# ACMEAtronOmatic/DSen2

Hardware: AMD Instinct MI355X
Metric: 32x32x6 patches/sec (DSen2_20, d=6, batch 512) (higher is better)
Workload: dtype f32; 1 GPU; DSen2_20 d=6 F=128 fp32, 512 synthetic 32x32 patches (4+6 bands) per GPU per step, he_uniform random-init weights; batch_per_gpu=512, parallelism=patch-sharded dp1, backend=rccl, output_gather=False

## Files before the change

### dsen2_amd/_lib.py

```python
import ctypes
import os
import sys

_HERE = os.path.dirname(os.path.abspath(__file__))
LIB_PATH = os.environ.get('DSEN2_HIP_LIB') or os.path.join(_HERE, 'libdsen2_hip.so')

OK = 0
ERR_INVALID, ERR_HIP, ERR_NO_WEIGHTS, ERR_WORKSPACE, ERR_NO_DEVICE, ERR_NOMEM, ERR_INTERNAL = -1, -2, -3, -4, -5, -6, -7
DTYPE_U16, DTYPE_F32 = 0, 1
DTYPE_F64 = 2
MASK_BLANK_MAP = 3

c_float_p = ctypes.POINTER(ctypes.c_float)
c_int_p = ctypes.POINTER(ctypes.c_int)
c_void_p = ctypes.c_void_p
c_int = ctypes.c_int
c_size_t = ctypes.c_size_t
c_double = ctypes.c_double


class CorpusTile(ctypes.Structure):
    _fields_ = [('dev_lr10', c_void_p), ('dev_lr20', c_void_p), ('dev_lr60', c_void_p), ('dev_gt', c_void_p),
                ('grid_h', c_int), ('grid_w', c_int), ('gt_dtype', c_int)]


SIGNATURES = {
    'dsen2_version': (ctypes.c_char_p, []),
    'dsen2_last_error': (ctypes.c_char_p, []),
    'dsen2_device_count': (c_int, []),
    'dsen2_model_create': (c_int, [ctypes.POINTER(c_void_p), c_int, c_int, c_int, c_int, c_int, c_int]),
    'dsen2_model_destroy': (None, [c_void_p]),
    'dsen2_model_num_params': (c_size_t, [c_void_p]),
    'dsen2_model_load_weights': (c_int, [c_void_p, c_float_p, c_size_t]),
    'dsen2_model_workspace_bytes': (c_int, [c_void_p, c_int, c_int, c_int, ctypes.POINTER(c_size_t)]),
    'dsen2_model_forward': (c_int, [c_void_p, c_void_p, c_void_p, c_void_p, c_void_p, c_int, c_int, c_int,
                                    c_void_p, c_size_t, c_void_p]),
    'dsen2_model_body_launches': (c_int, [c_void_p, c_int, c_int, c_int]),
    'dsen2_dihedral_nchw': (c_int, [c_void_p, c_void_p, c_int, c_int, c_int, c_int, c_int, c_void_p, c_int, c_void_p]),
    'dsen2_dihedral_accumulate': (c_int, [c_void_p, c_void_p, c_int, c_int, c_int, c_int, c_int, c_int, c_void_p]),
    'dsen2_model_ensemble_workspace_bytes': (c_int, [c_void_p, c_int, c_int, c_int, c_int, ctypes.POINTER(c_size_t)]),
    'dsen2_model_forward_ensemble': (c_int, [c_void_p, c_void_p, c_void_p, c_void_p, c_void_p, c_int, c_int, c_int, c_int,
                                             c_void_p, c_size_t, c_void_p]),
    'dsen2_model_forward_timed': (c_int, [c_void_p, c_void_p, c_void_p, c_void_p, c_void_p, c_int, c_int, c_int,
                                          c_void_p, c_size_t, c_void_p, c_int, c_float_p]),
    'dsen2_model_forward_profile': (c_int, [c_void_p, c_void_p, c_void_p, c_void_p, c_void_p, c_int, c_int, c_int,
                                            c_void_p, c_size_t, c_void_p, c_int, c_int, c_float_p]),
    'dsen2_conv3x3_nhwc': (c_int, [c_void_p, c_float_p, c_float_p, c_void_p, c_void_p, c_int, c_int, c_int, c_int,
                                   c_int, c_int, ctypes.c_float, c_void_p]),
    'dsen2_conv3x3_nhwc_ref': (c_int, [c_void_p, c_float_p, c_float_p, c_void_p, c_void_p, c_int, c_int, c_int, c_int,
                                       c_int, c_int, ctypes.c_float, c_void_p]),
    'dsen2_split_f32': (c_int, [c_void_p, c_void_p, c_void_p, c_int, c_int, c_int, c_int, c_void_p]),
    'dsen2_join_f32': (c_int, [c_void_p, c_void_p, c_void_p, c_int, c_int, c_int, c_int, c_void_p]),
# ... 142 lines not shown
```

### dsen2_amd/asm_contract.py

```python
import os
import re
import subprocess
import tempfile

HERE = os.path.dirname(os.path.abspath(__file__))
CSRC = os.path.join(HERE, 'csrc')
DMA_SOURCES = ['conv3x3_body32.hip', 'conv3x3_body16w.hip']


class AsmContractError(RuntimeError):
    pass


def _code_lines(text):
    return [ln.strip() for ln in text.splitlines() if ln.strip() and not ln.strip().startswith((';', '.', '//'))]


def _kernels(text):
    out, name, body = {}, None, []
    for ln in text.splitlines():
        m = re.match(r'^(_Z\w+):', ln)
        if m:
            name, body = m.group(1), []
            continue
# ... 97 lines not shown
            n_dma = [sum(1 for ln in c if ln.startswith('buffer_load_dword') and ln.endswith('lds')) for c in copies]
            need(min(n_dma) == 0 and max(n_dma) > 0, 'kernel %s: DMAs in both copies of the item loop' % name, n_dma)
            quiet, loud = (copies[0], copies[1]) if n_dma[0] == 0 else (copies[1], copies[0])
            need(not any(re.search(r'\bm0\b', ln) for ln in quiet), 'kernel %s: M0 use in the compute-only copy' % name)
            run = None
            for ln in loud:
                if re.match(r's_mov_b32 (s\d+|vcc_lo|vcc_hi), m0$', ln):
                    need(run is None, 'kernel %s: M0 saved twice in one DMA statement' % name)
                    run = 0
                elif ln.startswith('buffer_load_dword') and ln.endswith('lds'):
                    need(run is not None, 'kernel %s: DMA outside a statement that saves M0' % name)
                    run += 1
                elif run and not re.match(r'(s_mov_b32 m0, |s_nop 0$)', ln):
                    need(run in (2, 4), 'kernel %s: a DMA statement of %d instructions' % (name, run))
                    run = None
    if src == 'conv3x3_body16w.hip':
        expect = {0: (0, 32), 1: (64, 64), 3: (64, 64)}
        expect3 = {0: (0, 64), 1: (64, 96), 3: (64, 64)}

        def count(pattern, want, msg, product=lambda m: True):
            found = []
            for name, body in kernels.items():
                m = re.search(pattern, name)
                if not m or not product(m):
                    continue
                found.append(body)
                loads = sum(1 for ln in body if ln.startswith('buffer_load_dwordx4') and not ln.endswith('lds'))
                stores = sum(1 for ln in body if ln.startswith('buffer_store_dwordx4'))
                need((loads, stores) == want(m), msg(m) % (loads, stores, want(m)))
            return found
# ... 49 lines not shown
        need(not any(ln.startswith('global_store') for ln in body), 'kernel %s stores outside its buffer descriptors' % name)
        mf = [i for i, ln in enumerate(body) if ln.startswith('v_mfma')]
        need(mf, 'kernel %s has no MFMA' % name)
        x3 = 'ELb1EEE' in name
        floor = 24 if x3 else 16
        loop = body[mf[0]:]
        scat = [i for i, ln in enumerate(loop) if ln.startswith('ds_write_b16')]
        need(scat, 'kernel %s: no halo scatter after the first MFMA' % name)
        waits = [ln for ln in loop[:scat[-1]] if ln.startswith('s_waitcnt') and 'vmcnt' in ln]
        low = [ln for ln in waits if int(re.search(r'vmcnt\((\d+)\)', ln).group(1)) < floor]
        need(not low, 'kernel %s: a wait inside the tile loop drains the deferred stores (divergent branch in the loop body?)' % name, low[:4])
    return True


TRAFFIC_KERNELS = {
    'dsen2_20_fp32': ('conv3x3_body32.hip', r'conv3x3_body32_kernelILi128ELi128ELi0ELi0ELi0ELi4ELb1E'),
    'vdsen2_20_bf16': ('conv3x3_body16w.hip', r'conv3x3_body16w_chain_kernelILi128ELi256ELi0E'),
    'dsen2_20_bf16x3': ('conv3x3_body16w.hip', r'conv3x3_body16w_x3_chain_kernelILi64ELi128E'),
    'vdsen2_20_fp32': ('conv3x3_body32.hip', r'conv3x3_body32_kernelILi256ELi256ELi0ELi0ELi0ELi4ELb1E'),
    'dsen2_20_bf16': ('conv3x3_body16w.hip', r'conv3x3_body16w_chain_kernelILi64ELi128ELi0E'),
    'vdsen2_20_bf16x3': ('conv3x3_body16w.hip', r'conv3x3_body16w_x3_chain_kernelILi128ELi256E'),
}
ISA_JSON = os.path.join(HERE, 'kernel_isa.json')


def isa_hashes(text):
    import hashlib
    out = {}
    for name, body in _kernels(text).items():
        out[name] = hashlib.sha256('\n'.join(normalised(body)).encode()).hexdigest()
    return out
# ... 32 lines not shown
```

### dsen2_amd/csrc/capi.hip

```cpp

#include <chrono>
#include <cstdarg>
#include <cstdio>
#include <cstring>
#include <exception>
#include <new>
#include <vector>

#include "capi_internal.h"

using namespace dsen2;

namespace {

thread_local char g_err[512] = "";

#ifdef DSEN2_DIAG
Tuning g_diag_tuning;
unsigned long long* g_diag_stamps = nullptr;
#endif
Tuning default_tuning() {
#ifdef DSEN2_DIAG
  return g_diag_tuning;
#else
// ... 4 lines not shown
constexpr int kWarmLaunches = 24;

}

namespace dsen2 {
int fail(int code, const char* fmt, ...) {
  va_list ap;
  va_start(ap, fmt);
  vsnprintf(g_err, sizeof(g_err), fmt, ap);
  va_end(ap);
  return code;
}
}

static bool may_chain(const dsen2_model* m) {
  return m->chain_stride != 0 && m->tune.chain && m->tune.grid_cap == 0 && (m->precision == 1 || m->tune.ablate == 0);
}

static int first_layer(const dsen2_model* m, const float* x10, const float* x20, const float* x60, int n, int h, int w,
                       const ForwardWs& B, bool x0_packed, hipStream_t stream) {
  const Layer& L = m->layers[0];
  const ConvPlan& pl = L.plan;
  const float* P = m->dev_params;
  const bool x3 = m->precision == 2 && m->num_layers > 0;
  ConvParams pf = make_params(B.x0, L.weights(P), L.bias(P), nullptr, B.a, n, h, w, 0, 0.f);
  if (pl.epilogue == kEpiReluSplit) {
    pf.out = reinterpret_cast<float*>(B.s0);
    pf.out2 = B.s1;
  }
  const FirstInputs fi{x60, m->c10, m->c20, m->c60};
  ConvParams pd = pf;
// ... 81 lines not shown

int forward_launches(const dsen2_model* m, const float* x10, const float* x20, const float* x60, float* out, int n, int h, int w,
                     const ForwardWs& B, size_t keep_step, bool x0_packed, hipStream_t stream, const hipEvent_t* ev) {
  const float* P = m->dev_params;
  const int d = m->num_layers;
  if (ev) HIP_TRY(hipEventRecord(ev[0], stream));
  if (int rc = first_layer(m, x10, x20, x60, n, h, w, B, x0_packed, stream)) return rc;
  if (ev) HIP_TRY(hipEventRecord(ev[1], stream));
  if (m->precision != 0 && d > 0) {
    if (keep_step > 0) {
      HIP_TRY((m->precision == 2 ? launch_join3_f32 : launch_join_f32)(B.s0, B.s1, B.x0f, n, h, w, m->feat, stream));
      HIP_TRY(hipMemcpyAsync(B.xkeep, B.s0, operand16_bytes(m, n, h, w), hipMemcpyDeviceToDevice, stream));
    }
    if (int rc = body16(m, B.s0, B.s1, B.t16, B.a, n, h, w, stream, keep_step, B.xkeep)) return rc;
  } else {
    for (int l = 1; l <= d; ++l) {
      const Layer& LA = m->layers[2 * l - 1];
      const Layer& LB = m->layers[2 * l];
      const float* x_in = B.a + (size_t)(l - 1) * keep_step;
      float* t = B.t + (size_t)(l - 1) * keep_step;
      HIP_TRY(launch(LA.plan, make_params(x_in, LA.weights(P), LA.bias(P), nullptr, t, n, h, w, 0, 0.f), LA.plan.epilogue, m->tune, stream));
      HIP_TRY(launch(LB.plan, make_params(t, LB.weights(P), LB.bias(P), x_in, B.a + (size_t)l * keep_step, n, h, w, 0, 0.1f),
                     LB.plan.epilogue, m->tune, stream));
    }
  }
  if (ev) HIP_TRY(hipEventRecord(ev[2], stream));
  {
    const Layer& L = m->layers.back();
    const float* skip = m->c60 > 0 ? x60 : x20;
    const float* x_d = B.a + (m->precision == 0 ? (size_t)d * keep_step : 0);
    ConvParams po = make_params(x_d, L.weights(P), L.bias(P), skip, out, n, h, w, m->cout, 0.f);
// ... 355 lines not shown
}

int dsen2_model_forward(dsen2_model* m, const float* x10, const float* x20, const float* x60, float* out, int n, int h, int w,
                        void* workspace, size_t workspace_bytes, void* stream) {
  return guarded([&] { return forward(m, x10, x20, x60, out, n, h, w, workspace, workspace_bytes, stream, nullptr); });
}

int dsen2_model_body_launches(const dsen2_model* m, int n, int h, int w) {
  return guarded([&]() -> int {
    if (!m) return fail(DSEN2_ERR_INVALID, "NULL model");
    if (int rc = check_shape(m, n, h, w)) return rc;
    if (int rc = check_device(m)) return rc;
    int dev = 0, cus = 0;
    if (hipGetDevice(&dev) != hipSuccess || hipDeviceGetAttribute(&cus, hipDeviceAttributeMultiprocessorCount, dev) != hipSuccess)
      return fail(DSEN2_ERR_NO_DEVICE, "no HIP device");
    return may_chain(m) && body16w_chain_patches_per_wg(n, h, w, m->feat, cus) > 0 ? 1 : 2 * m->num_layers;
  });
}

int dsen2_model_forward_timed(dsen2_model* m, const float* x10, const float* x20, const float* x60, float* out, int n, int h, int w,
                              void* workspace, size_t workspace_bytes, void* stream, int iters, float* body_ms_per_launch) {
  return guarded([&]() -> int {
    if (!body_ms_per_launch) return fail(DSEN2_ERR_INVALID, "NULL result");
    if (!m || m->num_layers <= 0) return fail(DSEN2_ERR_INVALID, "model has no residual blocks");
    float ms[5];
    int rc = forward_profile(m, x10, x20, x60, out, n, h, w, workspace, workspace_bytes, stream, 0, iters, ms);
    if (rc == DSEN2_OK) *body_ms_per_launch = ms[2] / (2.0f * m->num_layers);
    return rc;
  });
}

int dsen2_model_forward_profile(dsen2_model* m, const float* x10, const float* x20, const float* x60, float* out, int n, int h,
// ... 208 lines not shown
```

### dsen2_amd/csrc/conv3x3_body32.hip

```cpp
#include <type_traits>

#include "conv3x3_dma.h"

namespace dsen2 {

namespace {

using dma::KC; using dma::NT; using dma::THREADS; using dma::QS; using dma::IN_BYTES; using dma::IN_BLOCKS;
using dma::WCH; using dma::NWBUF; using dma::LDS_BYTES; using dma::wait_vmcnt;
constexpr int KSTEPS = 4;
constexpr int PB = 2, MB = 2;
static_assert((8 * kHalo) % 16 == 0, "rows R and R+8 of a pixel block sit on the same banks");

}

template <int CIN, int COUT, int EPI, int ABL, int PRE, int STG, bool DEFER>
__global__ __launch_bounds__(THREADS, 2) void conv3x3_body32_kernel(const ConvParams p, const int n_items) {
  constexpr int NCC = CIN / KC;
  constexpr int NS = COUT / NT;
  static_assert(NCC % 2 == 0, "input double buffer parity");
  constexpr bool ASYM = STG >= 2;
  using Stage = dma::Stage<CIN, NS, false, ASYM ? dma::Role::Issuer : dma::Role::All>;
  constexpr int N_W = (ABL & 4) ? 0 : Stage::N_W;

// ... 246 lines not shown
    } else {
      if constexpr ((STG - 2) / KSTEPS == 1) __builtin_amdgcn_s_setprio(1);
      run(std::integral_constant<int, 0>{}, std::false_type{});
    }
  } else if constexpr (STG == 1) {
    if (wave < 4)
      run(std::integral_constant<int, 0>{}, std::true_type{});
    else
      run(std::integral_constant<int, KSTEPS / 2>{}, std::true_type{});
  } else {
    run(std::integral_constant<int, 0>{}, std::true_type{});
  }
  wait_vmcnt<0>();
}

template <int CIN, int COUT, int EPI, int ABL = 0, int PRE = 0, int STG = 0, bool DEFER = false>
static hipError_t launch_body32_one(const ConvParams& p, hipStream_t stream) {
  const long long items = (long long)p.n * p.tiles_x * p.tiles_y * (COUT / NT);
  return launch_persistent<conv3x3_body32_kernel<CIN, COUT, EPI, ABL, PRE, STG, DEFER>>(LDS_BYTES, THREADS, items, 1, 0, stream, p);
}

constexpr int kAsym = 2 + KSTEPS / 2;

template <int F>
static hipError_t launch_body32_feat(const ConvParams& p, int epilogue, Body32Form form, hipStream_t stream) {
  const bool relu = epilogue == kEpiRelu;
#ifdef DSEN2_DIAG
  if (form == Body32Form::Plain || form == Body32Form::StaggerA) {
    if (!relu) return launch_body32_one<F, F, kEpiResidual, 0, 2, 0>(p, stream);
    return form == Body32Form::Plain ? launch_body32_one<F, F, kEpiRelu, 0, 0, 0>(p, stream) : launch_body32_one<F, F, kEpiRelu, 0, 0, 1>(p, stream);
  }
  if (form == Body32Form::DeferStaggerA && !relu) return launch_body32_one<F, F, kEpiResidual, 0, 0, 0, true>(p, stream);
  if (form == Body32Form::DeferStagger || form == Body32Form::DeferStaggerA)
    return relu ? launch_body32_one<F, F, kEpiRelu, 0, 0, 1, true>(p, stream) : launch_body32_one<F, F, kEpiResidual, 0, 0, 1, true>(p, stream);
#define DSEN2_ASYM(FORM, STG)                                                                                      \
  if (form == Body32Form::FORM)                                                                                    \
    return relu ? launch_body32_one<F, F, kEpiRelu, 0, 0, STG, true>(p, stream) : launch_body32_one<F, F, kEpiResidual, 0, 0, STG, true>(p, stream);
// ... 35 lines not shown
```

### dsen2_amd/csrc/conv3x3_dma.h

```cpp
#pragma once
#include "conv3x3_items.h"

namespace dsen2 {
namespace dma {

constexpr int KC = 32;
constexpr int NT = 128;
constexpr int THREADS = 512;
constexpr int QS = 336;
constexpr int IN_BYTES = 8 * QS * 16;
constexpr int IN_BLOCKS = 6;
constexpr int WCH = KC * NT;
constexpr int NWBUF = 4;
constexpr size_t LDS_BYTES = (size_t)2 * IN_BYTES + (size_t)NWBUF * WCH * 4 + 256 * 4;
static_assert(QS >= kHaloPix && QS % 16 == 0 && 64 * (IN_BLOCKS - 1) + 16 == QS, "input chunk geometry");
static_assert(LDS_BYTES <= 160 * 1024, "LDS budget");

template <int N>
__device__ __forceinline__ void wait_vmcnt() {
  static_assert(N >= 0 && N <= 63, "vmcnt is a 6-bit field");
  asm volatile("s_waitcnt vmcnt(%0)" ::"n"(N) : "memory");
}

__device__ __forceinline__ unsigned lds_address(const float* p) {
  return (unsigned)(size_t)(__attribute__((address_space(3))) const float*)p;
}

enum class Role { All, Issuer };

template <int CINW, int NS, bool LAZY_VOFF = false, Role ROLE = Role::All>
struct Stage {
// ... 23 lines not shown
    in_rsrc = __builtin_amdgcn_make_buffer_rsrc(const_cast<float*>(p.in), 0, 0, 0x00020000);
    w_rsrc = __builtin_amdgcn_make_buffer_rsrc(const_cast<float*>(p.wpk), 0, (unsigned)(NS * NCHUNK * WCH * 4), 0x00020000);
    w_voff = lane * 16;
    wl_item = lid; wl_chunk = 0; st_slot = 0;
    st_y0 = st_x0 = 0;
  }

  __device__ __forceinline__ unsigned voff_of(int b, int ty0, int tx0) const {
    const int hp = 64 * b + lane;
    const int hy = hp / kHalo, hx = hp - hy * kHalo;
    const int gy = ty0 - 1 + hy, gx = tx0 - 1 + hx;
    const bool inb = hp < kHaloPix && (unsigned)gy < (unsigned)h && (unsigned)gx < (unsigned)w;
    return inb ? (unsigned)(((gy * w + gx) * CINW + wave * 4) * 4) : 0x80000000u;
  }

  __device__ __forceinline__ void set_stage_item(int item) {
    const Tile t = tile_at<NS>(item, tiles_per_img, tiles_x);
    in_rsrc = __builtin_amdgcn_make_buffer_rsrc(const_cast<float*>(in) + (size_t)t.img * img_pix * CINW, 0,
                                                (unsigned)(img_pix * CINW * 4), 0x00020000);
    if constexpr (LAZY_VOFF) {
      st_y0 = t.ty0;
      st_x0 = t.tx0;
    } else {
#pragma unroll
      for (int b = 0; b < IN_BLOCKS; ++b) in_voff[b] = voff_of(b, t.ty0, t.tx0);
    }
  }

  __device__ __forceinline__ void issue_in(int buf, int b, int cc) {
    const unsigned m0v = lds_in + buf * IN_BYTES + (wave * QS + 64 * b) * 16;
    const unsigned so = cc * (KC * 4);
    const unsigned voff = LAZY_VOFF ? voff_of(b, st_y0, st_x0) : in_voff[LAZY_VOFF ? 0 : b];
    if constexpr (ROLE == Role::Issuer) {
// ... 13 lines not shown
                     : "=&s"(saved_m0) : "s"(m0v), "s"(m1v), "v"(voff), "s"(in_rsrc), "s"(so), "s"(so1) : "memory");
      }
      return;
    }
    unsigned saved_m0;
    if (b < IN_BLOCKS - 1) {
      asm volatile("s_mov_b32 %0, m0\n\ts_mov_b32 m0, %1\n\ts_nop 0\n\tbuffer_load_dwordx4 %2, %3, %4 offen lds\n\ts_mov_b32 m0, %0"
                   : "=&s"(saved_m0) : "s"(m0v), "v"(voff), "s"(in_rsrc), "s"(so) : "memory");
    } else if (lane < 16) {
      asm volatile("s_mov_b32 %0, m0\n\ts_mov_b32 m0, %1\n\ts_nop 0\n\tbuffer_load_dwordx4 %2, %3, %4 offen lds\n\ts_mov_b32 m0, %0"
                   : "=&s"(saved_m0) : "s"(m0v), "v"(voff), "s"(in_rsrc), "s"(so) : "memory");
    }
  }

  __device__ __forceinline__ void issue_w() {
    const unsigned so = (unsigned)(((wl_item % NS) * NCHUNK + wl_chunk) * (WCH * 4) + wave * 1024);
    const unsigned l0 = lds_w + st_slot * (WCH * 4) + wave * 1024;
    unsigned saved_m0;
    if constexpr (ROLE == Role::Issuer)
      asm volatile(
          "s_mov_b32 %0, m0\n\t"
          "s_mov_b32 m0, %1\n\ts_nop 0\n\tbuffer_load_dwordx4 %5, %6, %7 offen lds\n\t"
          "s_mov_b32 m0, %2\n\ts_nop 0\n\tbuffer_load_dwordx4 %5, %6, %8 offen lds\n\t"
          "s_mov_b32 m0, %3\n\ts_nop 0\n\tbuffer_load_dwordx4 %5, %6, %9 offen lds\n\t"
          "s_mov_b32 m0, %4\n\ts_nop 0\n\tbuffer_load_dwordx4 %5, %6, %10 offen lds\n\t"
          "s_mov_b32 m0, %0"
          : "=&s"(saved_m0)
          : "s"(l0), "s"(l0 + 4096u), "s"(l0 + 8192u), "s"(l0 + 12288u), "v"(w_voff), "s"(w_rsrc), "s"(so), "s"(so + 4096u),
            "s"(so + 8192u), "s"(so + 12288u)
          : "memory");
    else
    asm volatile(
        "s_mov_b32 %0, m0\n\t"
        "s_mov_b32 m0, %1\n\ts_nop 0\n\tbuffer_load_dwordx4 %3, %4, %5 offen lds\n\t"
        "s_mov_b32 m0, %2\n\ts_nop 0\n\tbuffer_load_dwordx4 %3, %4, %6 offen lds\n\t"
        "s_mov_b32 m0, %0"
        : "=&s"(saved_m0) : "s"(l0), "s"(l0 + 8192u), "v"(w_voff), "s"(w_rsrc), "s"(so), "s"(so + 8192u)
        : "memory");
    if (++wl_chunk == NCHUNK) {
      wl_chunk = 0;
      wl_item = wl_item + G < n_items ? wl_item + G : lid;
    }
    st_slot = st_slot == NWBUF - 1 ? 0 : st_slot + 1;
  }
};

}
}
```

### dsen2_amd/csrc/conv_plan.h

```cpp
#pragma once
#include <vector>

#include "dsen2_internal.h"

namespace dsen2 {

enum class ConvRole { First, BodyA, BodyB, Output, DgradBody, DgradOutput };
enum class ConvKernel {
  Tile,
  Body32,
  Body16,
  Body16x3,
  Out
};

constexpr size_t kAlignFloats = 64;
inline size_t align_up(size_t v) { return (v + kAlignFloats - 1) / kAlignFloats * kAlignFloats; }

struct ConvPlan {
  ConvRole role;
  ConvKernel kernel;
  int epilogue;
  int cin, cout;
  int cin_pad, cout_pad;
// ... 15 lines not shown

struct Layer {
  ConvPlan plan;
  size_t off, flat_off;
  const float* weights(const float* params) const { return params + off; }
  const float* bias(const float* params) const { return params + off + plan.bias_off; }
  const float* first16(const float* params) const { return params + off + plan.first16_off; }
};
struct NetworkPlan {
  std::vector<Layer> layers;
  size_t n_params = 0;
  size_t dev_param_floats = 0;
  size_t chain_stride = 0;
};
bool plan_network(int c10, int c20, int c60, int num_layers, int feat, int precision, const Tuning& tune, NetworkPlan* net);

}
```

### dsen2_amd/csrc/conv_plan.hip

```cpp
#include <cstring>
#include <vector>

#include "conv_plan.h"

namespace dsen2 {

namespace {

constexpr int kBody16Chunk = 32;

bool sentinel2(const BandGroups* b) { return b && b->c10 == 4 && b->c20 == 6 && (b->c60 == 0 || b->c60 == 2); }

void pack_tile_weights(const float* k, const ConvPlan& pl, float* dst) {
  const int ncc = pl.cin_pad / pl.kc, nslab = pl.cout_pad / pl.nt, ng = pl.kc / 4;
  size_t i = 0;
  for (int slab = 0; slab < nslab; ++slab)
    for (int cc = 0; cc < ncc; ++cc)
      for (int tap = 0; tap < 9; ++tap)
        for (int gg = 0; gg < ng; ++gg)
          for (int o = 0; o < pl.nt; ++o)
            for (int j = 0; j < 4; ++j, ++i) {
              const int c = cc * pl.kc + 4 * gg + j, oc = slab * pl.nt + o;
              dst[i] = (c < pl.cin && oc < pl.cout) ? k[((size_t)tap * pl.cin + c) * pl.cout + oc] : 0.f;
            }
// ... 75 lines not shown
      pl.kernel = precision == 1   ? ConvKernel::Body16
                  : precision == 2 ? ConvKernel::Body16x3
                  : tune.body == BodyKernel::Body32 ? ConvKernel::Body32 : ConvKernel::Tile;
      break;
  }
  const size_t taps = tap_floats(pl);
  pl.weight_floats = pl.kernel == ConvKernel::Body16     ? taps / 2
                     : pl.kernel == ConvKernel::Body16x3 ? 3 * taps / 2
                                                         : taps + (pl.out_mfma ? out_mfma_weight_floats(cin) : 0);
  pl.bias_off = align_up(pl.weight_floats);
  pl.floats = pl.first16_off = pl.bias_off + align_up((size_t)pl.cout_pad);
  if (pl.first16_planes) pl.floats += align_up((first16_weight_u16(cout, pl.first16_planes == 2) + 1) / 2);
  return true;
}

void pack(const ConvPlan& pl, const float* k, const float* bias, float* dst) {
  memset(dst, 0, sizeof(float) * (bias ? pl.floats : pl.weight_floats));
  switch (pl.kernel) {
    case ConvKernel::Tile:
    case ConvKernel::Body32: pack_tile_weights(k, pl, dst); break;
    case ConvKernel::Body16: pack_conv_weights_bf16_host(k, pl.cin, pl.cout, reinterpret_cast<uint16_t*>(dst)); break;
    case ConvKernel::Body16x3: pack_conv_weights_bf16x3_host(k, pl.cin, pl.cout, reinterpret_cast<uint16_t*>(dst)); break;
    case ConvKernel::Out:
      pack_out_valu_weights_host(k, pl.cin, pl.cout, dst);
      if (pl.out_mfma) pack_out_mfma_weights_host(k, pl.cin, pl.cout, dst + tap_floats(pl));
      break;
  }
  if (!bias) return;
  memcpy(dst + pl.bias_off, bias, sizeof(float) * pl.cout);
  if (pl.first16_planes)
// ... 26 lines not shown
  *net = NetworkPlan{};
  auto add = [&](ConvRole role, int ci, int co, int prec) {
    Layer L;
    if (!plan_conv(role, ci, co, prec, tune, &bands, &L.plan)) return false;
    L.flat_off = net->n_params;
    net->n_params += (size_t)9 * ci * co + co;
    L.off = net->dev_param_floats;
    net->dev_param_floats += L.plan.floats;
    net->layers.push_back(L);
    return true;
  };
  if (!add(ConvRole::First, c10 + c20 + c60, feat, num_layers > 0 ? precision : 0)) return false;
  for (int i = 0; i < num_layers; ++i)
    if (!add(ConvRole::BodyA, feat, feat, precision) || !add(ConvRole::BodyB, feat, feat, precision)) return false;
  if (!add(ConvRole::Output, feat, c60 > 0 ? c60 : c20, 0)) return false;
  if (num_layers > 0 && precision != 0) net->chain_stride = net->layers[1].plan.floats * sizeof(float);
  return true;
}

}
```

### dsen2_amd/csrc/dsen2_internal.h

```cpp
#pragma once
#include <hip/hip_runtime.h>
#include <stddef.h>
#include <stdint.h>

#include <mutex>

namespace dsen2 {


constexpr int kTile = 16;
constexpr int kHalo = kTile + 2;
constexpr int kHaloPix = kHalo * kHalo;

enum Epilogue : int {
  kEpiRelu = 0, kEpiResidual = 1, kEpiSkipNCHW = 2,
  kEpiResidualF32 = 3,
  kEpiReluSplit = 4
};

struct ConvParams {
  const float* in;
  const float* wpk;
  const float* bias;
  const float* aux;
// ... 62 lines not shown
hipError_t launch_conv3x3_body16w(const ConvParams& p, int feat, int epilogue, bool x3, int ablate, hipStream_t stream, int grid_cap = 0);
hipError_t launch_split3_f32(const float* in_nhwc, void* hx, void* lo, int n, int h, int w, int c, hipStream_t stream);
struct ChainArgs {
  void* hi;
  void* lo;
  void* t;
  float* out_f32;
  unsigned layer_stride;
  int n_layers;
  int patches_per_wg;
  int seamless;
};
hipError_t launch_conv3x3_body16w_chain(const ConvParams& p, const ChainArgs& c, int feat, hipStream_t stream, int ablate = 0,
                                        bool x3 = false);
int body16w_chain_patches_per_wg(int n, int h, int w, int feat, int cus);
hipError_t launch_split_f32(const float* in_nhwc, void* hi, void* lo, int n, int h, int w, int c, hipStream_t stream);
hipError_t launch_join_f32(const void* hi, const void* lo, float* out_nhwc, int n, int h, int w, int c, hipStream_t stream);
inline uint16_t f32_to_bf16_rne(float f) {
  uint32_t u = __builtin_bit_cast(uint32_t, f);
  if ((u & 0x7fffffffu) > 0x7f800000u) return (uint16_t)((u >> 16) | 0x40);
  u += 0x7fffu + ((u >> 16) & 1u);
  return (uint16_t)(u >> 16);
}

hipError_t launch_pack_inputs(const float* x10, const float* x20, const float* x60, int c10, int c20, int c60,
                              float* out_nhwc16, int n, int h, int w, hipStream_t stream);
hipError_t launch_upsample(const float* in, float* out, int planes, int h, int w, int oh, int ow, float post_div,
                           hipStream_t stream, bool general = false);
hipError_t launch_tile_gather(const float* img, int H, int W, int C, int border, const int* origins, int count,
                              int P, float divisor, float* patches, hipStream_t stream);
// ... 65 lines not shown
```

### include/dsen2_hip.h

```cpp
#ifndef DSEN2_HIP_H
#define DSEN2_HIP_H

#include <stddef.h>

#ifdef __cplusplus
extern "C" {
#endif

#define DSEN2_OK 0
#define DSEN2_ERR_INVALID (-1)
#define DSEN2_ERR_HIP (-2)
#define DSEN2_ERR_NO_WEIGHTS (-3)
#define DSEN2_ERR_WORKSPACE (-4)
#define DSEN2_ERR_NO_DEVICE (-5)
#define DSEN2_ERR_NOMEM (-6)
#define DSEN2_ERR_INTERNAL (-7)

typedef struct dsen2_model dsen2_model;

const char *dsen2_version(void);
const char *dsen2_last_error(void);
int dsen2_device_count(void);

int dsen2_model_create(dsen2_model **out, int c10, int c20, int c60, int num_layers, int feature_size,
                       int precision);
void dsen2_model_destroy(dsen2_model *m);

size_t dsen2_model_num_params(const dsen2_model *m);

int dsen2_model_load_weights(dsen2_model *m, const float *host_flat, size_t count);

int dsen2_model_workspace_bytes(const dsen2_model *m, int n, int h, int w, size_t *bytes);

int dsen2_model_forward(dsen2_model *m, const float *dev_x10, const float *dev_x20, const float *dev_x60,
                        float *dev_out, int n, int h, int w, void *dev_workspace, size_t workspace_bytes,
                        void *stream);

int dsen2_model_body_launches(const dsen2_model *m, int n, int h, int w);

int dsen2_model_forward_timed(dsen2_model *m, const float *x10, const float *x20, const float *x60, float *out,
                              int n, int h, int w, void *workspace, size_t workspace_bytes, void *stream, int iters,
                              float *body_ms_per_launch);

int dsen2_model_forward_profile(dsen2_model *m, const float *x10, const float *x20, const float *x60, float *out,
                                int n, int h, int w, void *workspace, size_t workspace_bytes, void *stream, int warm,
                                int iters, float *ms5);

int dsen2_dihedral_nchw(const float *dev_in, float *dev_out, int n, int c, int h, int w, int op, const int *dev_ops_or_null,
                        int inverse, void *stream);
int dsen2_dihedral_accumulate(const float *dev_in, float *dev_acc, int n, int c, int h, int w, int op, int count_or_0,
                              void *stream);
int dsen2_model_ensemble_workspace_bytes(const dsen2_model *m, int n, int h, int w, int mask, size_t *bytes);
int dsen2_model_forward_ensemble(dsen2_model *m, const float *dev_x10, const float *dev_x20, const float *dev_x60,
// ... 165 lines not shown
```

Baseline: 40390 patches/s.

## Fuse fp32 residual-block body layers into one persistent chained kernel

Adds a persistent fp32 chain kernel that runs all 2*d body convolutions in a single launch. Each workgroup owns a fixed set of patches and walks layer by layer, ping-ponging activations between two buffers. It prefetches the next layer's weights and bias via LDS DMA while overlapping the previous item's epilogue (bias, ReLU or residual add) with the current MFMA loop. The aim is to remove per-layer launch overhead and tail imbalance for small 32x32 patches. The cost is that each workgroup must stay on its patches, so occupancy is limited to n/ppw workgroups, and the kernel is only enabled when the layout heuristic accepts it.

```diff
diff --git a/dsen2_amd/_lib.py b/dsen2_amd/_lib.py
--- a/dsen2_amd/_lib.py
+++ b/dsen2_amd/_lib.py
@@ -36,6 +36,7 @@
     'dsen2_model_forward': (c_int, [c_void_p, c_void_p, c_void_p, c_void_p, c_void_p, c_int, c_int, c_int,
                                     c_void_p, c_size_t, c_void_p]),
     'dsen2_model_body_launches': (c_int, [c_void_p, c_int, c_int, c_int]),
+    'dsen2_chain_patches_per_workgroup': (c_int, [c_int, c_int, c_int, c_int, c_int, c_int]),
     'dsen2_dihedral_nchw': (c_int, [c_void_p, c_void_p, c_int, c_int, c_int, c_int, c_int, c_void_p, c_int, c_void_p]),
     'dsen2_dihedral_accumulate': (c_int, [c_void_p, c_void_p, c_int, c_int, c_int, c_int, c_int, c_int, c_void_p]),
     'dsen2_model_ensemble_workspace_bytes': (c_int, [c_void_p, c_int, c_int, c_int, c_int, ctypes.POINTER(c_size_t)]),
diff --git a/dsen2_amd/asm_contract.py b/dsen2_amd/asm_contract.py
--- a/dsen2_amd/asm_contract.py
+++ b/dsen2_amd/asm_contract.py
@@ -135,6 +135,33 @@
                 elif run and not re.match(r'(s_mov_b32 m0, |s_nop 0$)', ln):
                     need(run in (2, 4), 'kernel %s: a DMA statement of %d instructions' % (name, run))
                     run = None
+        chains = {k: v for k, v in kernels.items() if re.search(r'conv3x3_body32_chain_kernelILi(128|256)E', k)}
+        need(len(chains) == 2, 'expected the 2 instantiations of the fp32 chain kernel, found %d' % len(chains))
+        for name, body in chains.items():
+            need(not any('scratch_' in ln or ln.startswith(('v_writelane_b32', 'v_readlane_b32')) for ln in body),
+                 'kernel %s spills registers' % name)
+            mf = [i for i, ln in enumerate(body) if ln.startswith('v_mfma')]
+            need(len(mf) == 2 * ITEM_MFMAS, 'kernel %s: %d MFMAs, expected two copies of the item loop' % (name, len(mf)))
+            copies = [body[mf[0]:mf[ITEM_MFMAS - 1]], body[mf[ITEM_MFMAS]:mf[-1]]]
+            n_dma = [sum(1 for ln in c if ln.startswith('buffer_load_dword') and ln.endswith('lds')) for c in copies]
+            need(min(n_dma) == 0 and max(n_dma) > 0, 'kernel %s: DMAs in both copies of the item loop' % name, n_dma)
+            quiet, loud = (copies[0], copies[1]) if n_dma[0] == 0 else (copies[1], copies[0])
+            need(not any(re.search(r'\bm0\b', ln) for ln in quiet), 'kernel %s: M0 use in the compute-only copy' % name)
+            need(any(ln.startswith('s_waitcnt') and re.search(r'vmcnt\(0\)', ln) for ln in quiet),
+                 'kernel %s: the compute-only copy never retires its own stores' % name)
+            run = None
+            for ln in loud:
+                if re.match(r's_mov_b32 (s\d+|vcc_lo|vcc_hi), m0$', ln):
+                    need(run is None, 'kernel %s: M0 saved twice in one DMA statement' % name)
+                    run = 0
+                elif ln.startswith('buffer_load_dword') and ln.endswith('lds'):
+                    need(run is not None, 'kernel %s: DMA outside a statement that saves M0' % name)
+                    run += 1
+                elif run and not re.match(r'(s_mov_b32 m0, |s_nop 0$)', ln):
+                    need(run in (1, 2, 4), 'kernel %s: a DMA statement of %d instructions' % (name, run))
+                    run = None
+            waits = [int(m.group(1)) for ln in loud for m in [re.search(r'^s_waitcnt vmcnt\((\d+)\)$', ln)] if m]
+            need(waits.count(6) >= 12 and waits.count(4) >= 6, 'kernel %s: the issuers\' counted step waits are gone' % name, waits[:20])
     if src == 'conv3x3_body16w.hip':
         expect = {0: (0, 32), 1: (64, 64), 3: (64, 64)}
         expect3 = {0: (0, 64), 1: (64, 96), 3: (64, 64)}
@@ -214,7 +241,7 @@
 
 
 TRAFFIC_KERNELS = {
-    'dsen2_20_fp32': ('conv3x3_body32.hip', r'conv3x3_body32_kernelILi128ELi128ELi0ELi0ELi0ELi4ELb1E'),
+    'dsen2_20_fp32': ('conv3x3_body32.hip', r'conv3x3_body32_chain_kernelILi128E'),
     'vdsen2_20_bf16': ('conv3x3_body16w.hip', r'conv3x3_body16w_chain_kernelILi128ELi256ELi0E'),
     'dsen2_20_bf16x3': ('conv3x3_body16w.hip', r'conv3x3_body16w_x3_chain_kernelILi64ELi128E'),
     'vdsen2_20_fp32': ('conv3x3_body32.hip', r'conv3x3_body32_kernelILi256ELi256ELi0ELi0ELi0ELi4ELb1E'),
diff --git a/dsen2_amd/csrc/capi.hip b/dsen2_amd/csrc/capi.hip
--- a/dsen2_amd/csrc/capi.hip
+++ b/dsen2_amd/csrc/capi.hip
@@ -42,7 +42,7 @@
 }
 
 static bool may_chain(const dsen2_model* m) {
-  return m->chain_stride != 0 && m->tune.chain && m->tune.grid_cap == 0 && (m->precision == 1 || m->tune.ablate == 0);
+  return m->num_layers > 0 && m->chain_stride != 0 && m->tune.chain && m->tune.grid_cap == 0 && (m->precision == 1 || m->tune.ablate == 0);
 }
 
 static int first_layer(const dsen2_model* m, const float* x10, const float* x20, const float* x60, int n, int h, int w,
@@ -154,7 +154,16 @@
     }
     if (int rc = body16(m, B.s0, B.s1, B.t16, B.a, n, h, w, stream, keep_step, B.xkeep)) return rc;
   } else {
-    for (int l = 1; l <= d; ++l) {
+    bool chained = false;
+    if (keep_step == 0 && may_chain(m)) {
+      const Layer& L1 = m->layers[1];
+      ChainArgs ca{};
+      ca.t = B.t; ca.out_f32 = B.a;
+      ca.layer_stride = (unsigned)m->chain_stride; ca.n_layers = 2 * d;
+      HIP_TRY(try_launch(launch_conv3x3_body32_chain(make_params(B.a, L1.weights(P), L1.bias(P), nullptr, nullptr, n, h, w, 0, 0.1f),
+                                                     ca, m->feat, stream), &chained));
+    }
+    for (int l = 1; l <= d && !chained; ++l) {
       const Layer& LA = m->layers[2 * l - 1];
       const Layer& LB = m->layers[2 * l];
       const float* x_in = B.a + (size_t)(l - 1) * keep_step;
@@ -540,8 +549,14 @@
     int dev = 0, cus = 0;
     if (hipGetDevice(&dev) != hipSuccess || hipDeviceGetAttribute(&cus, hipDeviceAttributeMultiprocessorCount, dev) != hipSuccess)
       return fail(DSEN2_ERR_NO_DEVICE, "no HIP device");
-    return may_chain(m) && body16w_chain_patches_per_wg(n, h, w, m->feat, cus) > 0 ? 1 : 2 * m->num_layers;
-  });
+    return may_chain(m) && chain_patches_per_wg(m->precision, n, h, w, m->feat, cus) > 0 ? 1 : 2 * m->num_layers;
+  });
+}
+
+int dsen2_chain_patches_per_workgroup(int precision, int feature_size, int n, int h, int w, int cus) {
+  if (precision < 0 || precision > 2 || (feature_size != 128 && feature_size != 256) || n <= 0 || h <= 0 || w <= 0 || cus <= 0)
+    return fail(DSEN2_ERR_INVALID, "bad argument");
+  return chain_patches_per_wg(precision, n, h, w, feature_size, cus);
 }
 
 int dsen2_model_forward_timed(dsen2_model* m, const float* x10, const float* x20, const float* x60, float* out, int n, int h, int w,
diff --git a/dsen2_amd/csrc/conv3x3_body32.hip b/dsen2_amd/csrc/conv3x3_body32.hip
--- a/dsen2_amd/csrc/conv3x3_body32.hip
+++ b/dsen2_amd/csrc/conv3x3_body32.hip
@@ -284,6 +284,246 @@
   wait_vmcnt<0>();
 }
 
+template <int F>
+constexpr unsigned kChainBiasOffset = 9u * F * F * 4u;
+
+template <int F>
+__global__ __launch_bounds__(THREADS, 2) void conv3x3_body32_chain_kernel(const ConvParams p, const ChainArgs chain) {
+  constexpr int NCC = F / KC;
+  constexpr int NS = F / NT;
+  static_assert(NCC % 2 == 0 && NCC >= 4, "input double buffer parity; a chunk between an item's epilogue and its successor's staging");
+  using Stage = dma::Stage<F, NS, false, dma::Role::Issuer>;
+  constexpr int N_W = Stage::N_W;
+
+  extern __shared__ __attribute__((aligned(16))) float smem[];
+  float* const in_s = smem;
+  float* const w_s = smem + 2 * IN_BYTES / 4;
+  float* const bias_s = w_s + NWBUF * WCH;
+
+  const int tid = threadIdx.x;
+  const int lane = tid & 63;
+  const int wave = __builtin_amdgcn_readfirstlane(tid >> 6);
+  const int wn = wave & 1;
+  const int wp = wave >> 1;
+  const int l31 = lane & 31;
+  const int hsel = lane >> 5;
+  const int rh = l31 >> 4, c16 = l31 & 15;
+
+  const int G = gridDim.x;
+  const int lid = xcd_contiguous_id(blockIdx.x, G);
+  const int tiles_per_img = p.tiles_x * p.tiles_y;
+  const int my_items = chain.patches_per_wg * tiles_per_img * NS;
+  const int item0 = lid * my_items;
+  const size_t img_pix = (size_t)p.h * p.w;
+  float* const ch_a = chain.out_f32;
+  float* const ch_t = reinterpret_cast<float*>(chain.t);
+
+  Stage st;
+  st.init(p, in_s, w_s, lane, wave, lid, G, 0);
+  st.span_layers(p, chain.layer_stride, chain.n_layers);
+  auto w_base = [&](int layer, int idx) -> unsigned {
+    return (unsigned)layer * chain.layer_stride + (unsigned)((idx % NS) * Stage::NCHUNK * (WCH * 4) + wave * 1024);
+  };
+
+  const int x_lane = (hsel * QS + (2 * wp + 8 * rh) * kHalo + c16) * 4;
+  const int w_lane = (hsel * NT + wn * 64 + l31) * 4;
+
+  if (wave < 4) {
+    st.set_stage_item(item0);
+#pragma unroll
+    for (int b = 0; b < IN_BLOCKS; ++b) st.issue_in(0, b, 0);
+#pragma unroll
+    for (int c = 0; c < NWBUF - 1; ++c) {
+      st.st_slot = c;
+      st.emit_w(w_base(0, 0) + c * (WCH * 4));
+    }
+  }
+  if (tid < F) bias_s[tid] = p.bias[tid];
+  wait_vmcnt<0>();
+  __syncthreads();
+
+  f32x4 w_cur[MB], x_cur[PB], w_nxt[MB], x_nxt[PB];
+  int mf_slot = 0;
+  auto read_frags = [&](f32x4 (&wf)[MB], f32x4 (&xf)[PB], const float* ib, const float* wb, int tap, int s) {
+    const int dy = tap / 3, dx = tap - dy * 3;
+    const float* wp_ = wb + w_lane + (2 * s * NT) * 4;
+    const float* xp_ = ib + x_lane + (2 * s * QS + dy * kHalo + dx) * 4;
+#pragma unroll
+    for (int mb = 0; mb < MB; ++mb) wf[mb] = *reinterpret_cast<const f32x4*>(wp_ + mb * 32 * 4);
+#pragma unroll
+    for (int pb = 0; pb < PB; ++pb) xf[pb] = *reinterpret_cast<const f32x4*>(xp_ + pb * kHalo * 4);
+  };
+  read_frags(w_cur, x_cur, in_s, w_s, 0, 0);
+
+  struct OutGeom { int img; unsigned lane_eoff; int ey; bool col_ok; int chb; };
+  auto out_geom = [&](int item, bool valid) -> OutGeom {
+    const Tile t = tile_at<NS>(item, tiles_per_img, p.tiles_x);
+    const int chb = t.slab * NT + wn * 64 + 4 * hsel;
+    const int ex = t.tx0 + c16, ey = t.ty0 + 2 * wp + 8 * rh;
+    return OutGeom{t.img, (unsigned)((ey * p.w + ex) * F + chb), ey, valid && ex < p.w, chb};
+  };
+  auto byte_off = [&](const OutGeom& g_, int mb, int pb, int g) -> unsigned {
+    return g_.col_ok && g_.ey + pb < p.h ? (g_.lane_eoff + (unsigned)(pb * p.w * F + mb * 32 + 8 * g)) * 4u : 0x80000000u;
+  };
+
+  auto run = [&](auto mid_c, auto issue_c) {
+  constexpr int MIDS = decltype(mid_c)::value;
+  constexpr bool ISSUE = decltype(issue_c)::value;
+  f32x16 acc[MB][PB];
+#pragma unroll
+  for (int mb = 0; mb < MB; ++mb)
+#pragma unroll
+    for (int pb = 0; pb < PB; ++pb)
+#pragma unroll
+      for (int e = 0; e < 16; ++e) acc[mb][pb][e] = 0.f;
+  f32x16 held[MB][PB];
+  f32x4 rq[4];
+#pragma unroll
+  for (int q = 0; q < 4; ++q) rq[q] = f32x4{0.f, 0.f, 0.f, 0.f};
+
+  int cur_layer = 0, cur_idx = 0;
+  for (;;) {
+    const bool loop_end = cur_layer == chain.n_layers;
+    const bool have_prev = (cur_layer | cur_idx) != 0;
+    const int prev_idx = cur_idx == 0 ? my_items - 1 : cur_idx - 1;
+    const int prev_layer = cur_idx == 0 ? cur_layer - 1 : cur_layer;
+    const OutGeom g_ = out_geom(have_prev ? item0 + prev_idx : item0, have_prev);
+    const int epi_b = __builtin_amdgcn_readfirstlane(have_prev ? prev_layer & 1 : 0);
+    const float* const bias_cur = bias_s + (prev_layer & 1) * F;
+    const auto out_rsrc = __builtin_amdgcn_make_buffer_rsrc(
+        (epi_b ? ch_a : ch_t) + (size_t)g_.img * img_pix * F, 0, (unsigned)(img_pix * F * 4), 0x00020000);
+    auto load_res = [&](int j) -> f32x4 {
+      const int mb = j >> 3, pb = (j >> 2) & 1, g = j & 3;
+      return __builtin_bit_cast(f32x4, __builtin_amdgcn_raw_buffer_load_b128(out_rsrc, byte_off(g_, mb, pb, g), 0, 0));
+    };
+    auto finish = [&](int j, const f32x16& a, f32x4 rr) {
+      const int mb = j >> 3, pb = (j >> 2) & 1, g = j & 3;
+      const f32x4 bias = *reinterpret_cast<const f32x4*>(bias_cur + g_.chb + mb * 32 + 8 * g);
+      f32x4 v = {a[4 * g], a[4 * g + 1], a[4 * g + 2], a[4 * g + 3]};
+      v = v + bias;
+      if (epi_b) {
+        v = rr + v * p.res_scale;
+      } else {
+#pragma unroll
+        for (int e = 0; e < 4; ++e) v[e] = fmaxf(v[e], 0.f);
+      }
+      __builtin_amdgcn_raw_buffer_store_b128(__builtin_bit_cast(u32x4, v), out_rsrc, byte_off(g_, mb, pb, g), 0, 0);
+    };
+#pragma unroll
+    for (int mb = 0; mb < MB; ++mb)
+#pragma unroll
+      for (int pb = 0; pb < PB; ++pb) held[mb][pb] = acc[mb][pb];
+    if (loop_end) {
+#pragma unroll
+      for (int j = 0; j < 16; ++j) {
+        f32x4 rr = {1.f, 1.f, 1.f, 1.f};
+        if (epi_b) rr = load_res(j);
+        finish(j, held[j >> 3][(j >> 2) & 1], rr);
+      }
+    } else if (epi_b) {
+      rq[0] = load_res(0);
+      rq[1] = load_res(1);
+    }
+    if (loop_end) break;
+    const bool layer_ends = cur_idx + 1 == my_items;
+    const int next_idx = layer_ends ? 0 : cur_idx + 1;
+    const int next_layer = layer_ends ? cur_layer + 1 : cur_layer;
+    const unsigned wb_cur = w_base(cur_layer, cur_idx);
+    const unsigned wb_next = w_base(next_layer < chain.n_layers ? next_layer : 0, next_idx);
+    if constexpr (ISSUE) {
+      if (cur_idx == 1 && cur_layer + 1 < chain.n_layers && wave < F / 64)
+        st.issue_dword(dma::lds_address(bias_s) + (unsigned)(((cur_layer + 1) & 1) * F * 4 + wave * 256), lane * 4,
+                       (unsigned)(cur_layer + 1) * chain.layer_stride + (unsigned)(kChainBiasOffset<F> + wave * 256));
+    }
+#pragma unroll
+    for (int mb = 0; mb < MB; ++mb)
+#pragma unroll
+      for (int pb = 0; pb < PB; ++pb)
+#pragma unroll
+        for (int e = 0; e < 16; ++e) acc[mb][pb][e] = 0.f;
+
+    auto do_cc = [&](const int cc, auto first_c) {
+      constexpr bool kFirst = decltype(first_c)::value;
+      (void)kFirst;
+      const float* const ib = in_s + (cc & 1) * (IN_BYTES / 4);
+      const float* const ib_next = in_s + ((cc + 1) & 1) * (IN_BYTES / 4);
+      const bool last_cc = cc == NCC - 1;
+      const int in_cc = last_cc ? 0 : cc + 1;
+      if constexpr (ISSUE) {
+        if (last_cc && next_layer < chain.n_layers) st.set_stage_item_of((next_layer & 1) ? ch_t : ch_a, item0 + next_idx);
+      }
+#pragma unroll
+      for (int tap = 0; tap < 9; ++tap) {
+        const float* const wb = w_s + mf_slot * WCH;
+        const int nx_slot = mf_slot == NWBUF - 1 ? 0 : mf_slot + 1;
+        const float* const wb_nx = w_s + nx_slot * WCH;
+        const int n_in = tap < IN_BLOCKS ? Stage::N_IN : 0;
+
+#pragma unroll
+        for (int s = 0; s < KSTEPS; ++s) {
+          if (s < KSTEPS - 1) {
+            read_frags(w_nxt, x_nxt, ib, wb, tap, s + 1);
+          } else if (tap < 8) {
+            read_frags(w_nxt, x_nxt, ib, wb_nx, tap + 1, 0);
+          } else {
+            read_frags(w_nxt, x_nxt, ib_next, wb_nx, 0, 0);
+          }
+          if (kFirst && tap < 7 && s == MIDS) {
+            if (epi_b) {
+              rq[2 * ((tap + 1) & 1)] = load_res(2 * tap + 2);
+              rq[2 * ((tap + 1) & 1) + 1] = load_res(2 * tap + 3);
+            }
+          }
+          if constexpr (ISSUE) {
+            if (s == MIDS) {
+              asm volatile("" : "+s"(st.lds_in));
+              if (n_in) st.issue_in((cc + 1) & 1, tap < IN_BLOCKS ? tap : 0, in_cc);
+              const int c = cc * 9 + tap + NWBUF - 1;
+              st.st_slot = (mf_slot + NWBUF - 1) % NWBUF;
+              st.emit_w(last_cc && tap + NWBUF - 1 >= 9 ? wb_next + (tap + NWBUF - 1 - 9) * (WCH * 4) : wb_cur + c * (WCH * 4));
+            }
+          }
+          if (kFirst && tap < 8 && (s == 1 || s == 3)) {
+            const int j = 2 * tap + (s >> 1);
+            finish(j, held[j >> 3][(j >> 2) & 1], rq[2 * (tap & 1) + (s >> 1)]);
+          }
+          __builtin_amdgcn_sched_barrier(0);
+#pragma unroll
+          for (int j = 0; j < 4; ++j)
+#pragma unroll
+            for (int mb = 0; mb < MB; ++mb)
+#pragma unroll
+              for (int pb = 0; pb < PB; ++pb)
+                acc[mb][pb] = __builtin_amdgcn_mfma_f32_32x32x2f32(w_cur[mb][j], x_cur[pb][j], acc[mb][pb], 0, 0, 0);
+#pragma unroll
+          for (int q = 0; q < MB; ++q) w_cur[q] = w_nxt[q];
+#pragma unroll
+          for (int q = 0; q < PB; ++q) x_cur[q] = x_nxt[q];
+        }
+        mf_slot = nx_slot;
+        __builtin_amdgcn_sched_barrier(0);
+        if constexpr (ISSUE) {
+          if (n_in) wait_vmcnt<N_W + Stage::N_IN>(); else wait_vmcnt<N_W>();
+        } else {
+          if (!kFirst && tap == 8) wait_vmcnt<0>();
+        }
+        __syncthreads();
+      }
+    };
+    do_cc(0, std::true_type{});
+#pragma unroll 1
+    for (int cc = 1; cc < NCC; ++cc) do_cc(cc, std::false_type{});
+    cur_layer = next_layer;
+    cur_idx = next_idx;
+  }
+  };
+  if (wave < 4)
+    run(std::integral_constant<int, KSTEPS / 2>{}, std::true_type{});
+  else
+    run(std::integral_constant<int, 0>{}, std::false_type{});
+  wait_vmcnt<0>();
+}
+
 template <int CIN, int COUT, int EPI, int ABL = 0, int PRE = 0, int STG = 0, bool DEFER = false>
 static hipError_t launch_body32_one(const ConvParams& p, hipStream_t stream) {
   const long long items = (long long)p.n * p.tiles_x * p.tiles_y * (COUT / NT);
@@ -291,6 +531,42 @@
 }
 
 constexpr int kAsym = 2 + KSTEPS / 2;
+
+constexpr int kChainMaxTilesPerPatch = 16;
+
+int body32_chain_patches_per_wg(int n, int h, int w, int feat, int cus) {
+  if (n <= 0 || h <= 0 || w <= 0 || cus <= 0 || (feat != 128 && feat != 256)) return 0;
+  const long long tiles = (long long)((w + kTile - 1) / kTile) * ((h + kTile - 1) / kTile);
+  if (tiles > kChainMaxTilesPerPatch) return 0;
+  const long long ipp = tiles * (feat / NT);
+  const int ppw = (n + cus - 1) / cus;
+  if (ppw < 2 || n % ppw != 0) return 0;
+  const long long rounds_layerwise = (n * ipp + cus - 1) / cus;
+  return ppw * ipp <= rounds_layerwise ? ppw : 0;
+}
+
+template <int F>
+static hipError_t launch_body32_chain_one(const ConvParams& p, ChainArgs c, hipStream_t stream) {
+  int cus = 0;
+  const hipError_t e = prepare_kernel<conv3x3_body32_chain_kernel<F>>(dma::LDS_BYTES_CHAIN, &cus);
+  if (e != hipSuccess) return e;
+  const long long bias_delta = reinterpret_cast<const char*>(p.bias) - reinterpret_cast<const char*>(p.wpk);
+  if (bias_delta != (long long)kChainBiasOffset<F> || bias_delta + F * 4 > (long long)c.layer_stride) return hipErrorInvalidValue;
+  if (c.n_layers < 2 || (c.n_layers & 1) || (unsigned long long)c.n_layers * c.layer_stride >= 0x80000000ull) return hipErrorInvalidValue;
+  c.patches_per_wg = body32_chain_patches_per_wg(p.n, p.h, p.w, F, cus);
+  if (c.patches_per_wg <= 0) return hipErrorNotSupported;
+  c.seamless = 1;
+  const int grid = p.n / c.patches_per_wg;
+  return launch_kernel<conv3x3_body32_chain_kernel<F>>(dim3(grid), THREADS, dma::LDS_BYTES_CHAIN, stream, p, c);
+}
+
+hipError_t launch_conv3x3_body32_chain(const ConvParams& p, const ChainArgs& c, int feat, hipStream_t stream) {
+  if (!p.in || !p.wpk || !p.bias || !c.t || !c.out_f32 || p.in != c.out_f32) return hipErrorInvalidValue;
+  if ((size_t)p.h * p.w * feat * 4 >= 0x80000000ull) return hipErrorNotSupported;
+  if (feat == 128) return launch_body32_chain_one<128>(p, c, stream);
+  if (feat == 256) return launch_body32_chain_one<256>(p, c, stream);
+  return hipErrorInvalidValue;
+}
 
 template <int F>
 static hipError_t launch_body32_feat(const ConvParams& p, int epilogue, Body32Form form, hipStream_t stream) {
diff --git a/dsen2_amd/csrc/conv3x3_dma.h b/dsen2_amd/csrc/conv3x3_dma.h
--- a/dsen2_amd/csrc/conv3x3_dma.h
+++ b/dsen2_amd/csrc/conv3x3_dma.h
@@ -13,8 +13,9 @@
 constexpr int WCH = KC * NT;
 constexpr int NWBUF = 4;
 constexpr size_t LDS_BYTES = (size_t)2 * IN_BYTES + (size_t)NWBUF * WCH * 4 + 256 * 4;
+constexpr size_t LDS_BYTES_CHAIN = LDS_BYTES + 256 * 4;
 static_assert(QS >= kHaloPix && QS % 16 == 0 && 64 * (IN_BLOCKS - 1) + 16 == QS, "input chunk geometry");
-static_assert(LDS_BYTES <= 160 * 1024, "LDS budget");
+static_assert(LDS_BYTES_CHAIN <= 160 * 1024, "LDS budget");
 
 template <int N>
 __device__ __forceinline__ void wait_vmcnt() {
@@ -68,9 +69,10 @@
     return inb ? (unsigned)(((gy * w + gx) * CINW + wave * 4) * 4) : 0x80000000u;
   }
 
-  __device__ __forceinline__ void set_stage_item(int item) {
+  __device__ __forceinline__ void set_stage_item(int item) { set_stage_item_of(in, item); }
+  __device__ __forceinline__ void set_stage_item_of(const float* src, int item) {
     const Tile t = tile_at<NS>(item, tiles_per_img, tiles_x);
-    in_rsrc = __builtin_amdgcn_make_buffer_rsrc(const_cast<float*>(in) + (size_t)t.img * img_pix * CINW, 0,
+    in_rsrc = __builtin_amdgcn_make_buffer_rsrc(const_cast<float*>(src) + (size_t)t.img * img_pix * CINW, 0,
                                                 (unsigned)(img_pix * CINW * 4), 0x00020000);
     if constexpr (LAZY_VOFF) {
       st_y0 = t.ty0;
@@ -114,7 +116,14 @@
   }
 
   __device__ __forceinline__ void issue_w() {
-    const unsigned so = (unsigned)(((wl_item % NS) * NCHUNK + wl_chunk) * (WCH * 4) + wave * 1024);
+    emit_w((unsigned)(((wl_item % NS) * NCHUNK + wl_chunk) * (WCH * 4) + wave * 1024));
+    if (++wl_chunk == NCHUNK) {
+      wl_chunk = 0;
+      wl_item = wl_item + G < n_items ? wl_item + G : lid;
+    }
+    st_slot = st_slot == NWBUF - 1 ? 0 : st_slot + 1;
+  }
+  __device__ __forceinline__ void emit_w(const unsigned so) {
     const unsigned l0 = lds_w + st_slot * (WCH * 4) + wave * 1024;
     unsigned saved_m0;
     if constexpr (ROLE == Role::Issuer)
@@ -137,11 +146,15 @@
         "s_mov_b32 m0, %0"
         : "=&s"(saved_m0) : "s"(l0), "s"(l0 + 8192u), "v"(w_voff), "s"(w_rsrc), "s"(so), "s"(so + 8192u)
         : "memory");
-    if (++wl_chunk == NCHUNK) {
-      wl_chunk = 0;
-      wl_item = wl_item + G < n_items ? wl_item + G : lid;
-    }
-    st_slot = st_slot == NWBUF - 1 ? 0 : st_slot + 1;
+  }
+
+  __device__ __forceinline__ void span_layers(const ConvParams& p, unsigned layer_stride, int n_layers) {
+    w_rsrc = __builtin_amdgcn_make_buffer_rsrc(const_cast<float*>(p.wpk), 0, (unsigned)n_layers * layer_stride, 0x00020000);
+  }
+  __device__ __forceinline__ void issue_dword(unsigned m0v, unsigned voff, unsigned soff) {
+    unsigned saved_m0;
+    asm volatile("s_mov_b32 %0, m0\n\ts_mov_b32 m0, %1\n\ts_nop 0\n\tbuffer_load_dword %2, %3, %4 offen lds\n\ts_mov_b32 m0, %0"
+                 : "=&s"(saved_m0) : "s"(m0v), "v"(voff), "s"(w_rsrc), "s"(soff) : "memory");
   }
 };
 
diff --git a/dsen2_amd/csrc/conv_plan.h b/dsen2_amd/csrc/conv_plan.h
--- a/dsen2_amd/csrc/conv_plan.h
+++ b/dsen2_amd/csrc/conv_plan.h
@@ -53,5 +53,6 @@
   size_t chain_stride = 0;
 };
 bool plan_network(int c10, int c20, int c60, int num_layers, int feat, int precision, const Tuning& tune, NetworkPlan* net);
+int chain_patches_per_wg(int precision, int n, int h, int w, int feat, int cus);
 
 }
diff --git a/dsen2_amd/csrc/conv_plan.hip b/dsen2_amd/csrc/conv_plan.hip
--- a/dsen2_amd/csrc/conv_plan.hip
+++ b/dsen2_amd/csrc/conv_plan.hip
@@ -113,6 +113,10 @@
   return true;
 }
 
+int chain_patches_per_wg(int precision, int n, int h, int w, int feat, int cus) {
+  return precision == 0 ? body32_chain_patches_per_wg(n, h, w, feat, cus) : body16w_chain_patches_per_wg(n, h, w, feat, cus);
+}
+
 void pack(const ConvPlan& pl, const float* k, const float* bias, float* dst) {
   memset(dst, 0, sizeof(float) * (bias ? pl.floats : pl.weight_floats));
   switch (pl.kernel) {
@@ -169,7 +173,8 @@
   for (int i = 0; i < num_layers; ++i)
     if (!add(ConvRole::BodyA, feat, feat, precision) || !add(ConvRole::BodyB, feat, feat, precision)) return false;
   if (!add(ConvRole::Output, feat, c60 > 0 ? c60 : c20, 0)) return false;
-  if (num_layers > 0 && precision != 0) net->chain_stride = net->layers[1].plan.floats * sizeof(float);
+  if (num_layers > 0 && (precision != 0 || (net->layers[1].plan.kernel == ConvKernel::Body32 && c60 == 0)))
+    net->chain_stride = net->layers[1].plan.floats * sizeof(float);
   return true;
 }
 
diff --git a/dsen2_amd/csrc/dsen2_internal.h b/dsen2_amd/csrc/dsen2_internal.h
--- a/dsen2_amd/csrc/dsen2_internal.h
+++ b/dsen2_amd/csrc/dsen2_internal.h
@@ -100,6 +100,8 @@
 hipError_t launch_conv3x3_body16w_chain(const ConvParams& p, const ChainArgs& c, int feat, hipStream_t stream, int ablate = 0,
                                         bool x3 = false);
 int body16w_chain_patches_per_wg(int n, int h, int w, int feat, int cus);
+hipError_t launch_conv3x3_body32_chain(const ConvParams& p, const ChainArgs& c, int feat, hipStream_t stream);
+int body32_chain_patches_per_wg(int n, int h, int w, int feat, int cus);
 hipError_t launch_split_f32(const float* in_nhwc, void* hi, void* lo, int n, int h, int w, int c, hipStream_t stream);
 hipError_t launch_join_f32(const void* hi, const void* lo, float* out_nhwc, int n, int h, int w, int c, hipStream_t stream);
 inline uint16_t f32_to_bf16_rne(float f) {
diff --git a/include/dsen2_hip.h b/include/dsen2_hip.h
--- a/include/dsen2_hip.h
+++ b/include/dsen2_hip.h
@@ -37,6 +37,8 @@
                         void *stream);
 
 int dsen2_model_body_launches(const dsen2_model *m, int n, int h, int w);
+
+int dsen2_chain_patches_per_workgroup(int precision, int feature_size, int n, int h, int w, int cus);
 
 int dsen2_model_forward_timed(dsen2_model *m, const float *x10, const float *x20, const float *x60, float *out,
                               int n, int h, int w, void *workspace, size_t workspace_bytes, void *stream, int iters,
```

Measured after the change: 40690 patches/s, median of 6. Within noise of the previous version (+0.8%).
